# lordzuko/SpeakingStyle

Hardware: AMD Instinct MI355X
Metric: train mel-frames/sec (node) (higher is better)
Workload: dtype bf16; 1 GPU; model=FastSpeech2 (LJSpeech model.yaml), global_batch=200, seq_len=T~LJSpeech phonemes, M<=1000 mel frames, parallelism=dp1

## Files before the change

csrc/build.py:

```python
#!/usr/bin/env python
import argparse
import concurrent.futures as cf
import glob
import os
import subprocess
import sys
import sysconfig

HERE = os.path.dirname(os.path.abspath(__file__))
ROOT = os.path.dirname(HERE)
OUT_DIR = os.path.join(ROOT, "speakingstyle_amd", "_lib")
OBJ_DIR = os.path.join(ROOT, "build", "obj")
KLIB = os.path.join(OUT_DIR, "libssamd_kernels.so")
HLIB = os.path.join(OUT_DIR, "libssamd_host.so")
FLIB = os.path.join(OUT_DIR, "ssamd_fast" + sysconfig.get_config_var("EXT_SUFFIX"))
ARCH = os.environ.get("SSAMD_ARCH", "gfx950")
HIPCC = os.environ.get("HIPCC", "/opt/rocm/bin/hipcc")


def _run(cmd):
    r = subprocess.run(cmd, stdout=subprocess.PIPE, stderr=subprocess.STDOUT, text=True)
    if r.returncode != 0:
        raise RuntimeError("command failed: %s\n%s" % (" ".join(cmd), r.stdout))
    return r.stdout
# ... 26 lines not shown
    if clean or _stale(KLIB, objs):
        _run([HIPCC, "-shared", f"--offload-arch={ARCH}", "-Wl,-soname,libssamd_kernels.so", "-o", KLIB] + objs)

    build_fastcall(clean)

    hsrcs = sorted(glob.glob(os.path.join(HERE, "host_*.cpp")))
    if hsrcs and (clean or _stale(HLIB, hsrcs + headers)):
        _run(["g++", "-O3", "-std=c++17", "-fPIC", "-shared", "-pthread", "-o", HLIB] + hsrcs)
    if verbose:
        print("built", KLIB, FLIB, HLIB if hsrcs else "")
    return KLIB


def build_fastcall(clean=False):
    sys.path.insert(0, ROOT)
    sys.path.insert(0, HERE)
    import gen_fastcall

    src = gen_fastcall.generate(*gen_fastcall.signatures())
    gen_dir = os.path.join(ROOT, "build", "gen")
    os.makedirs(gen_dir, exist_ok=True)
    cpp = os.path.join(gen_dir, "ssamd_fast.cpp")
    old = open(cpp).read() if os.path.exists(cpp) else None
    if old != src:
        with open(cpp, "w") as f:
            f.write(src)
    if clean or _stale(FLIB, [cpp, KLIB]):
        inc = sysconfig.get_paths()["include"]
        _run(["g++", "-O2", "-std=c++17", "-fPIC", "-shared", "-I", inc, "-o", FLIB, cpp, "-L", OUT_DIR,
              "-l:libssamd_kernels.so", "-Wl,-rpath,$ORIGIN"])
    return FLIB


SANITIZERS = {"asan": ["-fsanitize=address,undefined", "-fno-sanitize-recover=all", "-fno-omit-frame-pointer"],
              "tsan": ["-fsanitize=thread"]}


def build_sanitized(verbose=False):
    out_dir = os.path.join(ROOT, "build", "sanitize")
    os.makedirs(out_dir, exist_ok=True)
    hsrcs = sorted(glob.glob(os.path.join(HERE, "host_*.cpp")))
    test = os.path.join(HERE, "selftest_host_collate.cpp")
    exes = {}
    for name, flags in SANITIZERS.items():
        exe = os.path.join(out_dir, f"selftest_host_{name}")
        if _stale(exe, hsrcs + [test]):
            _run(["g++", "-O1", "-g", "-std=c++17", "-pthread"] + flags + ["-o", exe, test] + hsrcs)
        exes[name] = exe
    if verbose:
        print("built", " ".join(exes.values()))
    return exes


def build_blockmap_selftest():
    out_dir = os.path.join(ROOT, "build", "sanitize")
    os.makedirs(out_dir, exist_ok=True)
    test = os.path.join(HERE, "selftest_attn_blockmap.cpp")
    exe = os.path.join(out_dir, "selftest_attn_blockmap")
    if _stale(exe, [test, os.path.join(HERE, "attn_blockmap.h")]):
        _run(["g++", "-O1", "-g", "-std=c++17", "-I", HERE] + SANITIZERS["asan"] + ["-o", exe, test])
    return exe


def build_gl_selftest():
    out_dir = os.path.join(ROOT, "build", "sanitize")
    os.makedirs(out_dir, exist_ok=True)
    test = os.path.join(HERE, "selftest_gl_frames.cpp")
    exe = os.path.join(out_dir, "selftest_gl_frames")
    if _stale(exe, [test, os.path.join(HERE, "gl_frames.h")]):
        _run(["g++", "-O1", "-g", "-std=c++17", "-I", HERE] + SANITIZERS["asan"] + ["-o", exe, test])
    return exe


def build_dtw_selftest():
    out_dir = os.path.join(ROOT, "build", "sanitize")
    os.makedirs(out_dir, exist_ok=True)
    test = os.path.join(HERE, "selftest_dtw_index.cpp")
    exe = os.path.join(out_dir, "selftest_dtw_index")
    if _stale(exe, [test, os.path.join(HERE, "dtw_index.h")]):
        _run(["g++", "-O1", "-g", "-std=c++17", "-I", HERE] + SANITIZERS["asan"] + ["-o", exe, test])
    return exe


if __name__ == "__main__":
    ap = argparse.ArgumentParser()
    ap.add_argument("--jobs", type=int, default=min(8, os.cpu_count() or 4))
    ap.add_argument("--debug", action="store_true")
    ap.add_argument("--clean", action="store_true")
    ap.add_argument("--sanitize", action="store_true",
                    help="also build the host runtime self-test under ASan+UBSan and TSan (build/sanitize/)")
    a = ap.parse_args()
    try:
        build(a.jobs, a.debug, a.clean, verbose=True)
        if a.sanitize:
            build_sanitized(verbose=True)
    except RuntimeError as e:
        print(e, file=sys.stderr)
        sys.exit(1)
```

csrc/k_gemm.hip:

```cpp
#include <mutex>
#include "common.h"
#include <type_traits>

namespace {

constexpr int BM = 128, BN = 128, BK = 64;
constexpr int NT = 256;
constexpr int CSTRIDE = 132;

struct ConvGeom {
  int B, L, Cin, ks, dil, pad;
  int M, N, K;
  const int2* rinfo;
  const int64_t* cu;
  int nseq;
  int prio;
  int ngrp;
  int ksplit;
};

__device__ __forceinline__ int2 tile_of(int T, int nM, int nN, int ngrp) {
  if (ngrp > 1) {
    const int per = nN / ngrp, gs = nM * per;
    const int grp = T / gs, r = T - grp * gs;
    return make_int2(r / per, grp * per + r % per);
  }
  return make_int2(T / nN, T % nN);
}

__device__ __forceinline__ int2 row_pos(const ConvGeom& g, int m) {
  if (g.rinfo) return g.rinfo[m];
  const int b = m / g.L;
  return make_int2(m - b * g.L, g.L);
}

enum { ACT_NONE = 0, ACT_RELU = 1, ACT_LRELU = 2, ACT_TANH = 3 };

struct EpiX {
  const bf16_t* acc;
  bf16_t* y2;
  float scale;
  int post_act;
  const float* bn_stats;
  float* bn_part;
  float bn_p;
  unsigned long long bn_seed;
  unsigned char* mask_out;
  const unsigned char* mask_in;
};

__device__ __forceinline__ int xcd_remap(int bid, int nwg) {
  const int q = nwg / 8, r = nwg % 8, xcd = bid % 8, k = bid / 8;
  return (xcd < r ? xcd * (q + 1) : r * (q + 1) + (xcd - r) * q) + k;
}

__device__ __forceinline__ int swz128(int row, int c) { return row * 128 + ((c ^ ((row >> 1) & 7)) << 4); }

__device__ __forceinline__ short8 load_a_chunk(const bf16_t* __restrict__ X, const ConvGeom& g, int m, int tt, int lim,
                                               int k, float invCin) {
  short8 v = {0, 0, 0, 0, 0, 0, 0, 0};
  if (m < g.M && k < g.K) {
    const int tap = (int)(((float)k + 0.5f) * invCin);
    const int cin = k - tap * g.Cin;
    const int sh = tap * g.dil - g.pad;
    const int ts = tt + sh;
    if (ts >= 0 && ts < lim) v = *reinterpret_cast<const short8*>(X + ((long)m + sh) * g.Cin + cin);
  }
  return v;
}

template <bool OUT_F32>
__device__ __forceinline__ void epi4x4_prefetch(const float4v (&acc)[4][4], int mb, int nb, int lane, const ConvGeom& g,
                                                const float* __restrict__ bias, const bf16_t* __restrict__ aux,
                                                const bf16_t* __restrict__ resid, const int64_t* __restrict__ lens,
                                                int act, int ldy, void* __restrict__ Yv) {
  float4 bvj[4];
  short4v xa[4][4], xr[4][4];
  bool vrow[4];
#pragma unroll
  for (int j = 0; j < 4; ++j) {
    const int n = nb + j * 16 + 4 * (lane >> 4);
    bvj[j] = (bias && n < g.N) ? *reinterpret_cast<const float4*>(bias + n) : make_float4(0.f, 0.f, 0.f, 0.f);
  }
#pragma unroll
// ... 192 lines not shown
      if (aux) {
        short8 x = *reinterpret_cast<const short8*>(aux + off);
#pragma unroll
        for (int q = 0; q < 8; ++q) v[q] = bf2f((bf16_t)x[q]) > 0.f ? v[q] : 0.f;
      }
      if (resid) {
        short8 x = *reinterpret_cast<const short8*>(resid + off);
#pragma unroll
        for (int q = 0; q < 8; ++q) v[q] += bf2f((bf16_t)x[q]);
      }
      if (!valid) {
#pragma unroll
        for (int q = 0; q < 8; ++q) v[q] = 0.f;
      }
      if constexpr (OUT_F32) {
        float4* Y = reinterpret_cast<float4*>(reinterpret_cast<float*>(Yv) + off);
        Y[0] = make_float4(v[0], v[1], v[2], v[3]);
        Y[1] = make_float4(v[4], v[5], v[6], v[7]);
      } else {
        short8 o;
#pragma unroll
        for (int q = 0; q < 8; ++q) o[q] = (short)f2bf(v[q]);
        *reinterpret_cast<short8*>(reinterpret_cast<bf16_t*>(Yv) + off) = o;
      }
    } else {
      for (int q = 0; q < 8; ++q) {
        if (nb + q >= g.N) break;
        float x = v[q];
        if (aux && !(bf2f(aux[off + q]) > 0.f)) x = 0.f;
        if (resid) x += bf2f(resid[off + q]);
        if (!valid) x = 0.f;
        if constexpr (OUT_F32) reinterpret_cast<float*>(Yv)[off + q] = x;
        else reinterpret_cast<bf16_t*>(Yv)[off + q] = f2bf(x);
      }
    }
  }
}

__device__ __attribute__((aligned(16))) bf16_t g_zero_chunk_mem[8];
__device__ __forceinline__ const void* zero_chunk_ptr() {
  const void* p = g_zero_chunk_mem;
  asm volatile("" : "+s"(p));
  return p;
}

__device__ __forceinline__ void glds16(const void* src, char* lds_wave_base) {
  __builtin_amdgcn_global_load_lds((const __attribute__((address_space(1))) void*)src,
                                   (__attribute__((address_space(3))) void*)lds_wave_base, 16, 0, 0);
}
__device__ __forceinline__ void buf_lds16(__amdgpu_buffer_rsrc_t r, int voff, int soff, char* lds_wave_base) {
  __builtin_amdgcn_raw_ptr_buffer_load_lds(r, (__attribute__((address_space(3))) void*)lds_wave_base, 16, voff, soff,
                                           0, 0);
}

template <bool OUT_F32>
__global__ void __launch_bounds__(NT, 2) conv_gemm_glds_kernel(const bf16_t* __restrict__ X, const bf16_t* __restrict__ W,
                                                               const float* __restrict__ bias,
                                                               const bf16_t* __restrict__ aux,
                                                               const bf16_t* __restrict__ resid,
                                                               const int64_t* __restrict__ lens, void* __restrict__ Yv,
                                                               ConvGeom g, int act, int ldy) {
  const void* const g_zero_chunk = zero_chunk_ptr();
  extern __shared__ __attribute__((aligned(16))) char smem[];
  const int nN = (g.N + BN - 1) / BN;
  const int nM = (g.M + BM - 1) / BM;
  const int wg = xcd_remap(blockIdx.x, nN * nM);
  const int tn = wg % nN, tm = wg / nN;
  const int m0 = tm * BM, n0 = tn * BN;
  const int tid = threadIdx.x, lane = tid & 63, wave = __builtin_amdgcn_readfirstlane(tid >> 6);
  const int wm = wave >> 1, wn = wave & 1;
  const float invCin = 1.f / (float)g.Cin;

  int a_lim[4], a_t[4], a_m[4], rowi[4], lchunk[4];
#pragma unroll
  for (int i = 0; i < 4; ++i) {
    const int row = (i * 4 + wave) * 8 + (lane >> 3);
    rowi[i] = row;
    lchunk[i] = (lane & 7) ^ ((row >> 1) & 7);
    a_m[i] = m0 + row;
    const int2 rp = row_pos(g, a_m[i] < g.M ? a_m[i] : 0);
    a_t[i] = rp.x;
    a_lim[i] = rp.y;
  }
  auto stage = [&](int kt, int buf) {
    char* As = smem + buf * (2 * BM * BK * 2);
    char* Bs = As + BM * BK * 2;
#pragma unroll
    for (int i = 0; i < 4; ++i) {
      const int k = kt * BK + lchunk[i] * 8;
      const void* src = g_zero_chunk;
      if (a_m[i] < g.M && k < g.K) {
        const int tap = (int)(((float)k + 0.5f) * invCin);
        const int cin = k - tap * g.Cin;
        const int sh = tap * g.dil - g.pad;
        const int ts = a_t[i] + sh;
        if (ts >= 0 && ts < a_lim[i]) src = X + ((long)a_m[i] + sh) * g.Cin + cin;
      }
      glds16(src, As + (i * 4 + wave) * 8 * 128);
      const int n = n0 + rowi[i];
      const void* srcb = (n < g.N && k < g.K) ? (const void*)(W + (long)n * g.K + k) : (const void*)g_zero_chunk;
      glds16(srcb, Bs + (i * 4 + wave) * 8 * 128);
    }
  };

  float4v acc[4][4];
#pragma unroll
  for (int i = 0; i < 4; ++i)
#pragma unroll
    for (int j = 0; j < 4; ++j) acc[i][j] = (float4v){0.f, 0.f, 0.f, 0.f};

  const int nk = (g.K + BK - 1) / BK;
  stage(0, 0);
  asm volatile("s_waitcnt vmcnt(0)" ::: "memory");
  __syncthreads();
  for (int kt = 0; kt < nk; ++kt) {
    const int buf = kt & 1;
    if (kt + 1 < nk) stage(kt + 1, buf ^ 1);
    const char* As = smem + buf * (2 * BM * BK * 2);
    const char* Bs = As + BM * BK * 2;
#pragma unroll
    for (int kk = 0; kk < 2; ++kk) {
      short8 fa[4], fb[4];
      const int c = kk * 4 + (lane >> 4);
#pragma unroll
      for (int i = 0; i < 4; ++i) {
        fa[i] = *reinterpret_cast<const short8*>(As + swz128(wm * 64 + i * 16 + (lane & 15), c));
        fb[i] = *reinterpret_cast<const short8*>(Bs + swz128(wn * 64 + i * 16 + (lane & 15), c));
      }
#pragma unroll
      for (int i = 0; i < 4; ++i)
#pragma unroll
        for (int j = 0; j < 4; ++j) acc[i][j] = __builtin_amdgcn_mfma_f32_16x16x32_bf16(fb[j], fa[i], acc[i][j], 0, 0, 0);
    }
    asm volatile("s_waitcnt vmcnt(0)" ::: "memory");
    __syncthreads();
  }
  epi4x4_prefetch<OUT_F32>(acc, m0 + wm * 64, n0 + wn * 64, lane, g, bias, aux, resid, lens, act, ldy, Yv);
}

constexpr int BM3 = 256, NT3 = 512, NSTAGE = 3;
constexpr int STAGE_BYTES = (BM3 + BN) * BK * 2;

template <bool OUT_F32, bool FASTK, bool PACKED, bool BUF = false>
__global__ void __launch_bounds__(NT3, 1) conv_gemm_ring_kernel(const bf16_t* __restrict__ X, const bf16_t* __restrict__ W,
                                                                const float* __restrict__ bias,
                                                                const bf16_t* __restrict__ aux,
                                                                const bf16_t* __restrict__ resid,
                                                                const int64_t* __restrict__ lens, void* __restrict__ Yv,
                                                                ConvGeom g, int act, int ldy, EpiX ex) {
  const void* const g_zero_chunk = zero_chunk_ptr();
  extern __shared__ __attribute__((aligned(16))) char smem[];
  const int nN = (g.N + BN - 1) / BN;
  const int nM = (g.M + BM3 - 1) / BM3;
  const int wg = xcd_remap(blockIdx.x, nN * nM);
  const int tn = wg % nN, tm = wg / nN;
  const int m0 = tm * BM3, n0 = tn * BN;
  const int tid = threadIdx.x, lane = tid & 63, wave = __builtin_amdgcn_readfirstlane(tid >> 6);
  const int wm = wave >> 1, wn = wave & 1;
  const float invCin = 1.f / (float)g.Cin;

  int a_lim[4], a_t[4], a_m[4], achunk[4];
  const bf16_t* arow_ptr[4];
  const bf16_t* brow_ptr[2];
  bool a_ok[4], b_ok[2];
#pragma unroll
  for (int i = 0; i < 4; ++i) {
    const int row = (i * 8 + wave) * 8 + (lane >> 3);
    achunk[i] = (lane & 7) ^ ((row >> 1) & 7);
    a_m[i] = m0 + row;
    a_ok[i] = a_m[i] < g.M;
    const int mm = a_ok[i] ? a_m[i] : 0;
    if constexpr (PACKED) {
      const int2 rp = g.rinfo[mm];
      a_t[i] = rp.x;
      a_lim[i] = rp.y;
    } else {
      const int bb = mm / g.L;
      a_t[i] = mm - bb * g.L;
      a_lim[i] = g.L;
    }
    arow_ptr[i] = X + (long)mm * g.Cin + achunk[i] * 8;
  }
#pragma unroll
  for (int i = 0; i < 2; ++i) {
    const int row = (i * 8 + wave) * 8 + (lane >> 3);
    const int bch = (lane & 7) ^ ((row >> 1) & 7);
    const int n = n0 + row;
    b_ok[i] = n < g.N;
    brow_ptr[i] = W + (long)(b_ok[i] ? n : 0) * g.K + bch * 8;
  }
  constexpr int kOOB = (int)0x80000000;
  const __amdgpu_buffer_rsrc_t rA = __builtin_amdgcn_make_buffer_rsrc(
      (void*)(X - (long)g.pad * g.Cin), 0, BUF ? (g.M + g.pad) * g.Cin * 2 : 0, 0x00020000);
  const __amdgpu_buffer_rsrc_t rB = __builtin_amdgcn_make_buffer_rsrc((void*)W, 0, BUF ? g.N * g.K * 2 : 0,
                                                                      0x00020000);
  int avo[4], bvo[2];
  if constexpr (BUF) {
#pragma unroll
    for (int i = 0; i < 4; ++i) avo[i] = a_ok[i] ? ((a_m[i] + g.pad) * g.Cin + achunk[i] * 8) * 2 : kOOB;
#pragma unroll
    for (int i = 0; i < 2; ++i) {
      const int row = (i * 8 + wave) * 8 + (lane >> 3);
      const int bch = (lane & 7) ^ ((row >> 1) & 7);
      bvo[i] = b_ok[i] ? ((n0 + row) * g.K + bch * 8) * 2 : kOOB;
    }
  }
  auto stage = [&](int kt, int buf) {
    char* As = smem + buf * STAGE_BYTES;
    char* Bs = As + BM3 * BK * 2;
    const int k0 = kt * BK;
    if constexpr (BUF) {
      const int tap = k0 / g.Cin;
      const int cin0 = k0 - tap * g.Cin;
      const int shift = tap * g.dil - g.pad;
      const int aoff = (shift * g.Cin + cin0) * 2;
#pragma unroll
      for (int i = 0; i < 4; ++i) {
        const int ts = a_t[i] + shift;
        const bool ok = (unsigned)ts < (unsigned)a_lim[i];
        buf_lds16(rA, ok ? avo[i] + aoff : kOOB, 0, As + (i * 8 + wave) * 8 * 128);
      }
#pragma unroll
      for (int i = 0; i < 2; ++i) buf_lds16(rB, bvo[i], k0 * 2, Bs + (i * 8 + wave) * 8 * 128);
    } else if constexpr (FASTK) {
      const int tap = k0 / g.Cin;
      const int cin0 = k0 - tap * g.Cin;
      const int shift = tap * g.dil - g.pad;
      const long off = (long)shift * g.Cin + cin0;
#pragma unroll
      for (int i = 0; i < 4; ++i) {
        const int ts = a_t[i] + shift;
        const bool ok = a_ok[i] && (unsigned)ts < (unsigned)a_lim[i];
        glds16(ok ? (const void*)(arow_ptr[i] + off) : (const void*)g_zero_chunk, As + (i * 8 + wave) * 8 * 128);
      }
#pragma unroll
      for (int i = 0; i < 2; ++i)
        glds16(b_ok[i] ? (const void*)(brow_ptr[i] + k0) : (const void*)g_zero_chunk, Bs + (i * 8 + wave) * 8 * 128);
    } else {
#pragma unroll
      for (int i = 0; i < 4; ++i) {
        const int k = k0 + achunk[i] * 8;
        const void* src = g_zero_chunk;
        if (a_ok[i] && k < g.K) {
          const int tap = (int)(((float)k + 0.5f) * invCin);
          const int cin = k - tap * g.Cin;
          const int sh = tap * g.dil - g.pad;
          const int ts = a_t[i] + sh;
          if (ts >= 0 && ts < a_lim[i]) src = arow_ptr[i] - achunk[i] * 8 + (long)sh * g.Cin + cin;
        }
        glds16(src, As + (i * 8 + wave) * 8 * 128);
      }
#pragma unroll
      for (int i = 0; i < 2; ++i) {
        const int row = (i * 8 + wave) * 8 + (lane >> 3);
        const int k = k0 + ((lane & 7) ^ ((row >> 1) & 7)) * 8;
        glds16((b_ok[i] && k < g.K) ? (const void*)(brow_ptr[i] + k0) : (const void*)g_zero_chunk,
               Bs + (i * 8 + wave) * 8 * 128);
      }
    }
  };

  float4v acc[4][4];
#pragma unroll
  for (int i = 0; i < 4; ++i)
#pragma unroll
    for (int j = 0; j < 4; ++j) acc[i][j] = (float4v){0.f, 0.f, 0.f, 0.f};

  const int nk = (g.K + BK - 1) / BK;
  stage(0, 0);
  if (nk > 1) {
    stage(1, 1);
    asm volatile("s_waitcnt vmcnt(6)" ::: "memory");
  } else {
    asm volatile("s_waitcnt vmcnt(0)" ::: "memory");
  }
  __builtin_amdgcn_s_barrier();
  int buf = 0;
  for (int kt = 0; kt < nk; ++kt) {
    if (kt + 2 < nk) stage(kt + 2, (buf + 2) % NSTAGE);
    const char* As = smem + buf * STAGE_BYTES;
    const char* Bs = As + BM3 * BK * 2;
#pragma unroll
    for (int kk = 0; kk < 2; ++kk) {
      short8 fa[4], fb[4];
      const int c = kk * 4 + (lane >> 4);
#pragma unroll
      for (int i = 0; i < 4; ++i) {
        fa[i] = *reinterpret_cast<const short8*>(As + swz128(wm * 64 + i * 16 + (lane & 15), c));
        fb[i] = *reinterpret_cast<const short8*>(Bs + swz128(wn * 64 + i * 16 + (lane & 15), c));
      }
#pragma unroll
      for (int i = 0; i < 4; ++i)
#pragma unroll
        for (int j = 0; j < 4; ++j) acc[i][j] = __builtin_amdgcn_mfma_f32_16x16x32_bf16(fb[j], fa[i], acc[i][j], 0, 0, 0);
    }
    if (kt + 2 < nk) asm volatile("s_waitcnt vmcnt(6) lgkmcnt(0)" ::: "memory");
    else asm volatile("s_waitcnt vmcnt(0) lgkmcnt(0)" ::: "memory");
    __builtin_amdgcn_s_barrier();
    buf = (buf + 1) % NSTAGE;
  }
  float4 bvj[4];
  short4v xa[4][4], xr[4][4], xc[4][4];
  bool vrow[4];
#pragma unroll
  for (int j = 0; j < 4; ++j) {
    const int n = n0 + wn * 64 + j * 16 + 4 * (lane >> 4);
    bvj[j] = (bias && n < g.N) ? *reinterpret_cast<const float4*>(bias + n) : make_float4(0.f, 0.f, 0.f, 0.f);
  }
#pragma unroll
  for (int i = 0; i < 4; ++i) {
    const int m = m0 + wm * 64 + i * 16 + (lane & 15);
    const int mm = m < g.M ? m : 0;
    const int bb = mm / g.L, tt = mm - bb * g.L;
    vrow[i] = lens == nullptr || tt < (int)lens[bb];
#pragma unroll
    for (int j = 0; j < 4; ++j) {
      const int n = n0 + wn * 64 + j * 16 + 4 * (lane >> 4);
      const bool in = m < g.M && n < g.N;
      const long off = (long)m * ldy + n;
      if (in && aux) xa[i][j] = *reinterpret_cast<const short4v*>(aux + off);
// ... 108 lines not shown
    *reinterpret_cast<short4v*>(reinterpret_cast<bf16_t*>(Yv) + off) = o;
  }
}

constexpr int STG64_BYTES = 2 * BG * 64 * 2;
constexpr int B64_LDS = 256 * 528;

__device__ __forceinline__ void pp_barrier() {
  asm volatile("" ::: "memory");
  __builtin_amdgcn_sched_barrier(0);
  __builtin_amdgcn_s_barrier();
  __builtin_amdgcn_sched_barrier(0);
  asm volatile("" ::: "memory");
}

constexpr int EPI_GEN = 0, EPI_BNH = 1, EPI_MASK = 2;

__device__ __forceinline__ int ct_woff(int ml, int nl) { return ml * 528 + ((nl * 2) ^ (((ml >> 3) & 1) << 3)); }
__device__ __forceinline__ short8 ct_read(const char* Ct, int r, int c16) {
  const short8 v = *reinterpret_cast<const short8*>(Ct + r * 528 + c16 * 16);
  return ((r >> 3) & 1) ? __builtin_shufflevector(v, v, 4, 5, 6, 7, 0, 1, 2, 3) : v;
}
template <bool OUT_F32, bool FASTK, bool PACKED, bool BUF, int EPIM, bool STG>
__device__ __forceinline__ void big64_tile(const bf16_t* __restrict__ X, const bf16_t* __restrict__ W,
                                           const float* __restrict__ bias, const bf16_t* __restrict__ aux,
                                           const bf16_t* __restrict__ resid, const int64_t* __restrict__ lens,
                                           void* __restrict__ Yv, ConvGeom g, int act, int ldy, EpiX ex, int vb) {
  const void* const g_zero_chunk = zero_chunk_ptr();
  extern __shared__ __attribute__((aligned(16))) char smem[];
  const int nN = (g.N + BG - 1) / BG;
  const int nM = (g.M + BG - 1) / BG;
  const int2 tmn = tile_of(xcd_remap(vb, nN * nM), nM, nN, g.ngrp);
  const int tm = tmn.x, tn = tmn.y;
  const int m0 = tm * BG, n0 = tn * BG;
  const int tid = threadIdx.x, lane = tid & 63, wave = __builtin_amdgcn_readfirstlane(tid >> 6);
  const int wm = wave >> 2, wn = wave & 3;
  const float invCin = 1.f / (float)g.Cin;
  if (g.prio && wave >= 4) __builtin_amdgcn_s_setprio(1);

  int a_lim[4], a_t[4], a_m[4], achunk[4];
  const bf16_t* arow_ptr[4];
  const bf16_t* brow_ptr[4];
  bool a_ok[4], b_ok[4];
  int2 rp[4];
#pragma unroll
  for (int i = 0; i < 4; ++i) {
    const int row = (i * 8 + wave) * 8 + (lane >> 3);
    achunk[i] = (lane & 7) ^ ((row >> 1) & 7);
    a_m[i] = m0 + row;
    a_ok[i] = a_m[i] < g.M;
    if constexpr (PACKED) rp[i] = g.rinfo[a_ok[i] ? a_m[i] : 0];
  }
#pragma unroll
  for (int i = 0; i < 4; ++i) {
    const int mm = a_ok[i] ? a_m[i] : 0;
    if constexpr (PACKED) {
      a_t[i] = rp[i].x;
      a_lim[i] = rp[i].y;
    } else {
      const int bb = mm / g.L;
      a_t[i] = mm - bb * g.L;
      a_lim[i] = g.L;
    }
    arow_ptr[i] = X + (long)mm * g.Cin + achunk[i] * 8;
    const int row = (i * 8 + wave) * 8 + (lane >> 3);
    const int n = n0 + row;
    b_ok[i] = n < g.N;
    brow_ptr[i] = W + (long)(b_ok[i] ? n : 0) * g.K + achunk[i] * 8;
  }
  constexpr int kOOB = (int)0x80000000;
  const __amdgpu_buffer_rsrc_t rA = __builtin_amdgcn_make_buffer_rsrc(
      (void*)(X - (long)g.pad * g.Cin), 0, BUF ? (g.M + g.pad) * g.Cin * 2 : 0, 0x00020000);
  const __amdgpu_buffer_rsrc_t rB = __builtin_amdgcn_make_buffer_rsrc((void*)W, 0, BUF ? g.N * g.K * 2 : 0,
                                                                      0x00020000);
  int avo[4], bvo[4];
  if constexpr (BUF) {
#pragma unroll
    for (int i = 0; i < 4; ++i) {
      avo[i] = a_ok[i] ? ((a_m[i] + g.pad) * g.Cin + achunk[i] * 8) * 2 : kOOB;
      const int row = (i * 8 + wave) * 8 + (lane >> 3);
      bvo[i] = b_ok[i] ? ((n0 + row) * g.K + achunk[i] * 8) * 2 : kOOB;
    }
  }
  auto stage = [&](int kt, int buf) {
    char* As = smem + buf * STG64_BYTES;
    char* Bs = As + BG * 64 * 2;
    const int k0 = kt * 64;
    if constexpr (BUF) {
      const int tap = k0 / g.Cin;
      const int cin0 = k0 - tap * g.Cin;
      const int shift = tap * g.dil - g.pad;
      const int aoff = (shift * g.Cin + cin0) * 2;
#pragma unroll
      for (int i = 0; i < 4; ++i) {
        const int ts = a_t[i] + shift;
        const bool ok = (unsigned)ts < (unsigned)a_lim[i];
        buf_lds16(rA, ok ? avo[i] + aoff : kOOB, 0, As + (i * 8 + wave) * 1024);
      }
#pragma unroll
      for (int i = 0; i < 4; ++i) buf_lds16(rB, bvo[i], k0 * 2, Bs + (i * 8 + wave) * 1024);
    } else if constexpr (FASTK) {
      const int tap = k0 / g.Cin;
      const int cin0 = k0 - tap * g.Cin;
      const int shift = tap * g.dil - g.pad;
      const long off = (long)shift * g.Cin + cin0;
#pragma unroll
      for (int i = 0; i < 4; ++i) {
        const int ts = a_t[i] + shift;
        const bool ok = a_ok[i] && (unsigned)ts < (unsigned)a_lim[i];
        glds16(ok ? (const void*)(arow_ptr[i] + off) : (const void*)g_zero_chunk, As + (i * 8 + wave) * 1024);
      }
#pragma unroll
      for (int i = 0; i < 4; ++i)
        glds16(b_ok[i] ? (const void*)(brow_ptr[i] + k0) : (const void*)g_zero_chunk, Bs + (i * 8 + wave) * 1024);
    } else {
#pragma unroll
      for (int i = 0; i < 4; ++i) {
        const int k = k0 + achunk[i] * 8;
        const void* src = g_zero_chunk;
        if (a_ok[i] && k < g.K) {
          const int tap = (int)(((float)k + 0.5f) * invCin);
          const int cin = k - tap * g.Cin;
          const int sh = tap * g.dil - g.pad;
          const int ts = a_t[i] + sh;
          if (ts >= 0 && ts < a_lim[i]) src = arow_ptr[i] - achunk[i] * 8 + (long)sh * g.Cin + cin;
        }
        glds16(src, As + (i * 8 + wave) * 1024);
      }
#pragma unroll
      for (int i = 0; i < 4; ++i) {
        const int k = k0 + achunk[i] * 8;
        glds16((b_ok[i] && k < g.K) ? (const void*)(brow_ptr[i] + k0) : (const void*)g_zero_chunk,
               Bs + (i * 8 + wave) * 1024);
      }
    }
  };

  float4v acc[8][4];
#pragma unroll
  for (int i = 0; i < 8; ++i)
#pragma unroll
    for (int j = 0; j < 4; ++j) acc[i][j] = (float4v){0.f, 0.f, 0.f, 0.f};

  unsigned char mpre[16];
  if constexpr (EPIM == EPI_MASK) {
    const int c = tid & 31, r0 = tid >> 5;
    const int n = n0 + c * 8;
#pragma unroll
    for (int it = 0; it < 16; ++it) {
      const int m = m0 + r0 + 16 * it;
      mpre[it] = (n < g.N && m < g.M) ? ex.mask_in[(long)m * (g.N >> 3) + (n >> 3)] : (unsigned char)0;
    }
  }
  constexpr int BNH_PRE = STG ? 8 : 16;
  short8 hpre[16];
  auto load_h = [&](int it0, int it1) {
    const int c = tid & 31, r0 = tid >> 5;
    const int n = n0 + c * 8;
#pragma unroll
    for (int it = it0; it < it1; ++it) {
      const int m = m0 + r0 + 16 * it;
      hpre[it] = (short8){0, 0, 0, 0, 0, 0, 0, 0};
      if (n < g.N && m < g.M) hpre[it] = *reinterpret_cast<const short8*>(ex.acc + (long)m * ldy + n);
    }
  };
  if constexpr (EPIM == EPI_BNH) {
    load_h(0, BNH_PRE);
  }
  const int nk_all = (g.K + 63) / 64;
  int kt0 = 0, nk = nk_all;
  if (gridDim.y > 1) {
    const int per = (nk_all + gridDim.y - 1) / gridDim.y;
    kt0 = blockIdx.y * per;
    nk = min(nk_all, kt0 + per);
    Yv = reinterpret_cast<float*>(Yv) + (long)blockIdx.y * g.M * ldy;
  }
  if (g.ksplit > 0 && gridDim.y == 1) {
    const int kc = g.Cin / 64;
    if (n0 < g.ksplit) nk = 2 * kc;
    else kt0 = kc;
  }
  if constexpr (STG) {
    int bblk[4], bvo2[4];
    bblk[0] = 8 * (wave >> 2) + (wave & 3);
    bblk[1] = bblk[0] + 16;
    bblk[2] = bblk[0] + 4;
    bblk[3] = bblk[1] + 4;
#pragma unroll
    for (int u = 0; u < 4; ++u) {
      const int row = bblk[u] * 8 + (lane >> 3);
      const int ch = (lane & 7) ^ ((row >> 1) & 7);
      bvo2[u] = (n0 + row < g.N) ? ((n0 + row) * g.K + ch * 8) * 2 : kOOB;
    }
    auto stage_a = [&](int kt, int q, int buf) {
      char* As = smem + buf * STG64_BYTES;
      const int k0 = kt * 64;
      const int tap = k0 / g.Cin;
      const int cin0 = k0 - tap * g.Cin;
      const int shift = tap * g.dil - g.pad;
      const int aoff = (shift * g.Cin + cin0) * 2;
#pragma unroll
      for (int jj = 0; jj < 2; ++jj) {
        const int i = q + 2 * jj;
        const int ts = a_t[i] + shift;
        const bool ok = (unsigned)ts < (unsigned)a_lim[i];
        buf_lds16(rA, ok ? avo[i] + aoff : kOOB, 0, As + (i * 8 + wave) * 1024);
      }
    };
    auto stage_b = [&](int kt, int q, int buf) {
      char* Bs = smem + buf * STG64_BYTES + BG * 64 * 2;
#pragma unroll
      for (int jj = 0; jj < 2; ++jj) buf_lds16(rB, bvo2[q * 2 + jj], kt * 128, Bs + bblk[q * 2 + jj] * 1024);
    };
    short8 fa[2][4], fb0[2][2], fb1[2][2];
    auto read_a = [&](const char* As, int qa) {
#pragma unroll
      for (int kk = 0; kk < 2; ++kk) {
        const int c = kk * 4 + (lane >> 4);
#pragma unroll
        for (int i = 0; i < 4; ++i)
          fa[kk][i] = *reinterpret_cast<const short8*>(As + swz128(wm * 128 + qa * 64 + i * 16 + (lane & 15), c));
      }
    };
    auto read_b = [&](const char* Bs, int qb, short8 (&fb)[2][2]) {
#pragma unroll
      for (int kk = 0; kk < 2; ++kk) {
        const int c = kk * 4 + (lane >> 4);
#pragma unroll
        for (int j = 0; j < 2; ++j)
          fb[kk][j] = *reinterpret_cast<const short8*>(Bs + swz128(wn * 64 + qb * 32 + j * 16 + (lane & 15), c));
      }
    };
    auto mma = [&](int qa, int qb, const short8 (&fb)[2][2]) {
      asm volatile("s_waitcnt lgkmcnt(0)" ::: "memory");
      __builtin_amdgcn_sched_barrier(0);
      __builtin_amdgcn_s_setprio(1);
#pragma unroll
      for (int kk = 0; kk < 2; ++kk)
#pragma unroll
        for (int i = 0; i < 4; ++i)
#pragma unroll
          for (int j = 0; j < 2; ++j)
            acc[qa * 4 + i][qb * 2 + j] =
                __builtin_amdgcn_mfma_f32_16x16x32_bf16(fb[kk][j], fa[kk][i], acc[qa * 4 + i][qb * 2 + j], 0, 0, 0);
      __builtin_amdgcn_s_setprio(0);
    };
    const int nkt = nk - kt0;
    if (nkt > 0) { stage_a(kt0, 0, 0); stage_b(kt0, 1, 0); stage_a(kt0, 1, 0); stage_b(kt0, 0, 0); }
    if (nkt > 1) {
      stage_a(kt0 + 1, 0, 1); stage_b(kt0 + 1, 1, 1); stage_a(kt0 + 1, 1, 1); stage_b(kt0 + 1, 0, 1);
      asm volatile("s_waitcnt vmcnt(8)" ::: "memory");
    } else {
      asm volatile("s_waitcnt vmcnt(0)" ::: "memory");
    }
    pp_barrier();
    if (wm == 1) pp_barrier();
    for (int t = 0; t < nkt; ++t) {
      const int buf = t & 1, kt = kt0 + t;
      const char* As = smem + buf * STG64_BYTES;
      const char* Bs = As + BG * 64 * 2;
      const bool s1 = t >= 1 && t + 1 < nkt;
      const bool s2 = t + 2 < nkt;
      if (s1) stage_a(kt + 1, 1, buf ^ 1);
      read_a(As, 0);
      read_b(Bs, 0, fb0);
      pp_barrier();
      mma(0, 0, fb0);
      pp_barrier();
      if (s1) stage_b(kt + 1, 0, buf ^ 1);
      read_b(Bs, 1, fb1);
      pp_barrier();
      mma(0, 1, fb1);
      pp_barrier();
      if (s2) stage_a(kt + 2, 0, buf);
      read_a(As, 1);
      pp_barrier();
      mma(1, 1, fb1);
      pp_barrier();
      if (s2) stage_b(kt + 2, 1, buf);
      if (t + 1 < nkt) {
        if (s2) asm volatile("s_waitcnt vmcnt(4)" ::: "memory");
        else asm volatile("s_waitcnt vmcnt(0)" ::: "memory");
      }
      pp_barrier();
      mma(1, 0, fb0);
      pp_barrier();
    }
    if (wm == 0) pp_barrier();
    asm volatile("s_waitcnt vmcnt(0)" ::: "memory");
    pp_barrier();
  } else {
  if (kt0 < nk) stage(kt0, 0);
  asm volatile("s_waitcnt vmcnt(0)" ::: "memory");
  __builtin_amdgcn_s_barrier();
  for (int kt = kt0; kt < nk; ++kt) {
    const int buf = (kt - kt0) & 1;
    if (kt + 1 < nk) stage(kt + 1, buf ^ 1);
    const char* As = smem + buf * STG64_BYTES;
    const char* Bs = As + BG * 64 * 2;
#pragma unroll
    for (int kk = 0; kk < 2; ++kk) {
      const int c = kk * 4 + (lane >> 4);
      short8 fa[8], fb[4];
#pragma unroll
      for (int j = 0; j < 4; ++j) fb[j] = *reinterpret_cast<const short8*>(Bs + swz128(wn * 64 + j * 16 + (lane & 15), c));
#pragma unroll
      for (int i = 0; i < 8; ++i) fa[i] = *reinterpret_cast<const short8*>(As + swz128(wm * 128 + i * 16 + (lane & 15), c));
#pragma unroll
      for (int i = 0; i < 8; ++i)
#pragma unroll
        for (int j = 0; j < 4; ++j) acc[i][j] = __builtin_amdgcn_mfma_f32_16x16x32_bf16(fb[j], fa[i], acc[i][j], 0, 0, 0);
    }
    asm volatile("s_waitcnt vmcnt(0) lgkmcnt(0)" ::: "memory");
    __builtin_amdgcn_s_barrier();
  }
  }
  if constexpr (!OUT_F32) {
    if (act >= 0 && (g.N & 7) == 0 && (ldy & 7) == 0) {
      char* Ct = smem;
      auto stage_tile = [&](auto actc, auto biasc) {
        constexpr int A = decltype(actc)::value;
        constexpr bool HB = decltype(biasc)::value;
        float4 bv[4];
        if constexpr (HB) {
#pragma unroll
          for (int j = 0; j < 4; ++j) {
            const int n = n0 + wn * 64 + j * 16 + 4 * (lane >> 4);
            bv[j] = n < g.N ? *reinterpret_cast<const float4*>(bias + n) : make_float4(0.f, 0.f, 0.f, 0.f);
          }
        }
#pragma unroll
        for (int i = 0; i < 8; ++i) {
          const int ml = wm * 128 + i * 16 + (lane & 15);
#pragma unroll
          for (int j = 0; j < 4; ++j) {
            const int nl = wn * 64 + j * 16 + 4 * (lane >> 4);
            float v[4] = {acc[i][j][0], acc[i][j][1], acc[i][j][2], acc[i][j][3]};
            if constexpr (HB) {
              v[0] += bv[j].x; v[1] += bv[j].y; v[2] += bv[j].z; v[3] += bv[j].w;
            }
            if constexpr (A == ACT_RELU) {
#pragma unroll
              for (int q = 0; q < 4; ++q) v[q] = fmaxf(v[q], 0.f);
            } else if constexpr (A == ACT_LRELU) {
#pragma unroll
              for (int q = 0; q < 4; ++q) v[q] = v[q] > 0.f ? v[q] : 0.1f * v[q];
            } else if constexpr (A == ACT_TANH) {
#pragma unroll
              for (int q = 0; q < 4; ++q) v[q] = tanhf(v[q]);
            }
            short4v o;
#pragma unroll
            for (int q = 0; q < 4; ++q) o[q] = (short)f2bf(v[q]);
            *reinterpret_cast<short4v*>(Ct + ct_woff(ml, nl)) = o;
          }
        }
      };
      auto stage_act = [&](auto biasc) {
        if (act == ACT_RELU) stage_tile(std::integral_constant<int, ACT_RELU>{}, biasc);
        else if (act == ACT_LRELU) stage_tile(std::integral_constant<int, ACT_LRELU>{}, biasc);
        else if (act == ACT_TANH) stage_tile(std::integral_constant<int, ACT_TANH>{}, biasc);
        else stage_tile(std::integral_constant<int, ACT_NONE>{}, biasc);
      };
      if constexpr (EPIM == EPI_BNH) stage_tile(std::integral_constant<int, ACT_NONE>{}, std::false_type{});
      else if (bias) stage_act(std::true_type{});
      else stage_act(std::false_type{});
      if constexpr (EPIM == EPI_BNH) {
        if constexpr (BNH_PRE < 16) load_h(BNH_PRE, 16);
      }
// ... 1817 lines not shown
```

Before: 4.535 million mel-frames/s.

## Walk conv-GEMM K dimension chunk-major across taps to reuse activation rows

Adds a K-walk helper that orders the implicit-GEMM conv reduction chunk-major (all taps for one 64-channel chunk before moving on) unless ksplit needs tap-major order. It also adds a fast path in the generic stage that uses tap and chunk counters instead of float division per element, and advances slab counters incrementally in the pipelined kernel. Consecutive K steps then touch the same channel chunk of shifted activation rows, which is meant to improve cache reuse and cut the per-step index arithmetic. The accumulation order changes, so bf16/fp32 results may differ slightly. A host self-test for the walk is included.

```diff
diff --git a/csrc/build.py b/csrc/build.py
--- a/csrc/build.py
+++ b/csrc/build.py
@@ -132,6 +132,16 @@
     return exe
 
 
+def build_kwalk_selftest():
+    out_dir = os.path.join(ROOT, "build", "sanitize")
+    os.makedirs(out_dir, exist_ok=True)
+    test = os.path.join(HERE, "selftest_gemm_kwalk.cpp")
+    exe = os.path.join(out_dir, "selftest_gemm_kwalk")
+    if _stale(exe, [test, os.path.join(HERE, "gemm_kwalk.h")]):
+        _run(["g++", "-O1", "-g", "-std=c++17", "-I", HERE] + SANITIZERS["asan"] + ["-o", exe, test])
+    return exe
+
+
 if __name__ == "__main__":
     ap = argparse.ArgumentParser()
     ap.add_argument("--jobs", type=int, default=min(8, os.cpu_count() or 4))
diff --git a/csrc/gemm_kwalk.h b/csrc/gemm_kwalk.h
--- /dev/null
+++ b/csrc/gemm_kwalk.h
@@ -0,0 +1,54 @@
+#pragma once
+
+#if defined(__HIPCC__) || defined(__CUDACC__)
+#define KWALK_HD __host__ __device__
+#else
+#define KWALK_HD
+#endif
+
+#define KWALK_SLAB 64
+
+struct KSlab {
+  int tap;
+  int chunk;
+};
+
+KWALK_HD inline int kwalk_num_slabs(int Cin, int ks) { return ks * (Cin / KWALK_SLAB); }
+
+KWALK_HD inline KSlab kwalk_slab(int kt, int Cin, int ks, bool tap_major) {
+  KSlab s;
+  if (tap_major) {
+    const int kc = Cin / KWALK_SLAB;
+    s.tap = kt / kc;
+    s.chunk = kt - s.tap * kc;
+  } else {
+    s.chunk = kt / ks;
+    s.tap = kt - s.chunk * ks;
+  }
+  return s;
+}
+
+KWALK_HD inline KSlab kwalk_next(KSlab s, int Cin, int ks, bool tap_major) {
+  if (tap_major) {
+    if (++s.chunk == Cin / KWALK_SLAB) { s.chunk = 0; ++s.tap; }
+  } else {
+    if (++s.tap == ks) { s.tap = 0; ++s.chunk; }
+  }
+  return s;
+}
+
+KWALK_HD inline int kwalk_b_offset(KSlab s, int Cin) { return s.tap * Cin + s.chunk * KWALK_SLAB; }
+KWALK_HD inline int kwalk_a_shift(KSlab s, int dil, int pad) { return s.tap * dil - pad; }
+KWALK_HD inline int kwalk_a_channel(KSlab s) { return s.chunk * KWALK_SLAB; }
+
+KWALK_HD inline void kwalk_slice(int nk, int S, int y, int* kt0, int* kt1) {
+  const int per = (nk + S - 1) / S;
+  *kt0 = y * per < nk ? y * per : nk;
+  *kt1 = *kt0 + per < nk ? *kt0 + per : nk;
+}
+
+KWALK_HD inline void kwalk_ksplit_range(int Cin, bool low, int* kt0, int* kt1) {
+  const int kc = Cin / KWALK_SLAB;
+  *kt0 = low ? 0 : kc;
+  *kt1 = low ? 2 * kc : 3 * kc;
+}
diff --git a/csrc/k_gemm.hip b/csrc/k_gemm.hip
--- a/csrc/k_gemm.hip
+++ b/csrc/k_gemm.hip
@@ -1,5 +1,6 @@
 #include <mutex>
 #include "common.h"
+#include "gemm_kwalk.h"
 #include <type_traits>
 
 namespace {
@@ -358,9 +359,27 @@
     a_t[i] = rp.x;
     a_lim[i] = rp.y;
   }
+  const bool fastk = g.Cin % BK == 0;
   auto stage = [&](int kt, int buf) {
     char* As = smem + buf * (2 * BM * BK * 2);
     char* Bs = As + BM * BK * 2;
+    if (fastk) {
+      const KSlab sl = kwalk_slab(kt, g.Cin, g.ks, g.ksplit > 0);
+      const int shift = kwalk_a_shift(sl, g.dil, g.pad);
+      const long off = (long)shift * g.Cin + kwalk_a_channel(sl);
+      const int boff = kwalk_b_offset(sl, g.Cin);
+#pragma unroll
+      for (int i = 0; i < 4; ++i) {
+        const int ts = a_t[i] + shift;
+        const bool ok = a_m[i] < g.M && (unsigned)ts < (unsigned)a_lim[i];
+        glds16(ok ? (const void*)(X + (long)a_m[i] * g.Cin + off + lchunk[i] * 8) : g_zero_chunk,
+               As + (i * 4 + wave) * 8 * 128);
+        const int n = n0 + rowi[i];
+        glds16(n < g.N ? (const void*)(W + (long)n * g.K + boff + lchunk[i] * 8) : g_zero_chunk,
+               Bs + (i * 4 + wave) * 8 * 128);
+      }
+      return;
+    }
 #pragma unroll
     for (int i = 0; i < 4; ++i) {
       const int k = kt * BK + lchunk[i] * 8;
@@ -486,32 +505,32 @@
     char* Bs = As + BM3 * BK * 2;
     const int k0 = kt * BK;
     if constexpr (BUF) {
-      const int tap = k0 / g.Cin;
-      const int cin0 = k0 - tap * g.Cin;
-      const int shift = tap * g.dil - g.pad;
-      const int aoff = (shift * g.Cin + cin0) * 2;
+      const KSlab sl = kwalk_slab(kt, g.Cin, g.ks, g.ksplit > 0);
+      const int shift = kwalk_a_shift(sl, g.dil, g.pad);
+      const int aoff = (shift * g.Cin + kwalk_a_channel(sl)) * 2;
 #pragma unroll
       for (int i = 0; i < 4; ++i) {
         const int ts = a_t[i] + shift;
         const bool ok = (unsigned)ts < (unsigned)a_lim[i];
         buf_lds16(rA, ok ? avo[i] + aoff : kOOB, 0, As + (i * 8 + wave) * 8 * 128);
       }
-#pragma unroll
-      for (int i = 0; i < 2; ++i) buf_lds16(rB, bvo[i], k0 * 2, Bs + (i * 8 + wave) * 8 * 128);
+      const int boff = kwalk_b_offset(sl, g.Cin) * 2;
+#pragma unroll
+      for (int i = 0; i < 2; ++i) buf_lds16(rB, bvo[i], boff, Bs + (i * 8 + wave) * 8 * 128);
     } else if constexpr (FASTK) {
-      const int tap = k0 / g.Cin;
-      const int cin0 = k0 - tap * g.Cin;
-      const int shift = tap * g.dil - g.pad;
-      const long off = (long)shift * g.Cin + cin0;
+      const KSlab sl = kwalk_slab(kt, g.Cin, g.ks, g.ksplit > 0);
+      const int shift = kwalk_a_shift(sl, g.dil, g.pad);
+      const long off = (long)shift * g.Cin + kwalk_a_channel(sl);
 #pragma unroll
       for (int i = 0; i < 4; ++i) {
         const int ts = a_t[i] + shift;
         const bool ok = a_ok[i] && (unsigned)ts < (unsigned)a_lim[i];
         glds16(ok ? (const void*)(arow_ptr[i] + off) : (const void*)g_zero_chunk, As + (i * 8 + wave) * 8 * 128);
       }
+      const int boff = kwalk_b_offset(sl, g.Cin);
 #pragma unroll
       for (int i = 0; i < 2; ++i)
-        glds16(b_ok[i] ? (const void*)(brow_ptr[i] + k0) : (const void*)g_zero_chunk, Bs + (i * 8 + wave) * 8 * 128);
+        glds16(b_ok[i] ? (const void*)(brow_ptr[i] + boff) : (const void*)g_zero_chunk, Bs + (i * 8 + wave) * 8 * 128);
     } else {
 #pragma unroll
       for (int i = 0; i < 4; ++i) {
@@ -786,37 +805,38 @@
       bvo[i] = b_ok[i] ? ((n0 + row) * g.K + achunk[i] * 8) * 2 : kOOB;
     }
   }
+  const bool tapmaj = g.ksplit > 0;
   auto stage = [&](int kt, int buf) {
     char* As = smem + buf * STG64_BYTES;
     char* Bs = As + BG * 64 * 2;
     const int k0 = kt * 64;
     if constexpr (BUF) {
-      const int tap = k0 / g.Cin;
-      const int cin0 = k0 - tap * g.Cin;
-      const int shift = tap * g.dil - g.pad;
-      const int aoff = (shift * g.Cin + cin0) * 2;
+      const KSlab sl = kwalk_slab(kt, g.Cin, g.ks, tapmaj);
+      const int shift = kwalk_a_shift(sl, g.dil, g.pad);
+      const int aoff = (shift * g.Cin + kwalk_a_channel(sl)) * 2;
 #pragma unroll
       for (int i = 0; i < 4; ++i) {
         const int ts = a_t[i] + shift;
         const bool ok = (unsigned)ts < (unsigned)a_lim[i];
         buf_lds16(rA, ok ? avo[i] + aoff : kOOB, 0, As + (i * 8 + wave) * 1024);
       }
-#pragma unroll
-      for (int i = 0; i < 4; ++i) buf_lds16(rB, bvo[i], k0 * 2, Bs + (i * 8 + wave) * 1024);
+      const int boff = kwalk_b_offset(sl, g.Cin) * 2;
+#pragma unroll
+      for (int i = 0; i < 4; ++i) buf_lds16(rB, bvo[i], boff, Bs + (i * 8 + wave) * 1024);
     } else if constexpr (FASTK) {
-      const int tap = k0 / g.Cin;
-      const int cin0 = k0 - tap * g.Cin;
-      const int shift = tap * g.dil - g.pad;
-      const long off = (long)shift * g.Cin + cin0;
+      const KSlab sl = kwalk_slab(kt, g.Cin, g.ks, tapmaj);
+      const int shift = kwalk_a_shift(sl, g.dil, g.pad);
+      const long off = (long)shift * g.Cin + kwalk_a_channel(sl);
 #pragma unroll
       for (int i = 0; i < 4; ++i) {
         const int ts = a_t[i] + shift;
         const bool ok = a_ok[i] && (unsigned)ts < (unsigned)a_lim[i];
         glds16(ok ? (const void*)(arow_ptr[i] + off) : (const void*)g_zero_chunk, As + (i * 8 + wave) * 1024);
       }
+      const int boff = kwalk_b_offset(sl, g.Cin);
 #pragma unroll
       for (int i = 0; i < 4; ++i)
-        glds16(b_ok[i] ? (const void*)(brow_ptr[i] + k0) : (const void*)g_zero_chunk, Bs + (i * 8 + wave) * 1024);
+        glds16(b_ok[i] ? (const void*)(brow_ptr[i] + boff) : (const void*)g_zero_chunk, Bs + (i * 8 + wave) * 1024);
     } else {
 #pragma unroll
       for (int i = 0; i < 4; ++i) {
@@ -874,16 +894,10 @@
   const int nk_all = (g.K + 63) / 64;
   int kt0 = 0, nk = nk_all;
   if (gridDim.y > 1) {
-    const int per = (nk_all + gridDim.y - 1) / gridDim.y;
-    kt0 = blockIdx.y * per;
-    nk = min(nk_all, kt0 + per);
+    kwalk_slice(nk_all, gridDim.y, blockIdx.y, &kt0, &nk);
     Yv = reinterpret_cast<float*>(Yv) + (long)blockIdx.y * g.M * ldy;
   }
-  if (g.ksplit > 0 && gridDim.y == 1) {
-    const int kc = g.Cin / 64;
-    if (n0 < g.ksplit) nk = 2 * kc;
-    else kt0 = kc;
-  }
+  if (g.ksplit > 0 && gridDim.y == 1) kwalk_ksplit_range(g.Cin, n0 < g.ksplit, &kt0, &nk);
   if constexpr (STG) {
     int bblk[4], bvo2[4];
     bblk[0] = 8 * (wave >> 2) + (wave & 3);
@@ -896,13 +910,10 @@
       const int ch = (lane & 7) ^ ((row >> 1) & 7);
       bvo2[u] = (n0 + row < g.N) ? ((n0 + row) * g.K + ch * 8) * 2 : kOOB;
     }
-    auto stage_a = [&](int kt, int q, int buf) {
+    auto stage_a = [&](KSlab sl, int q, int buf) {
       char* As = smem + buf * STG64_BYTES;
-      const int k0 = kt * 64;
-      const int tap = k0 / g.Cin;
-      const int cin0 = k0 - tap * g.Cin;
-      const int shift = tap * g.dil - g.pad;
-      const int aoff = (shift * g.Cin + cin0) * 2;
+      const int shift = kwalk_a_shift(sl, g.dil, g.pad);
+      const int aoff = (shift * g.Cin + kwalk_a_channel(sl)) * 2;
 #pragma unroll
       for (int jj = 0; jj < 2; ++jj) {
         const int i = q + 2 * jj;
@@ -911,10 +922,11 @@
         buf_lds16(rA, ok ? avo[i] + aoff : kOOB, 0, As + (i * 8 + wave) * 1024);
       }
     };
-    auto stage_b = [&](int kt, int q, int buf) {
+    auto stage_b = [&](KSlab sl, int q, int buf) {
       char* Bs = smem + buf * STG64_BYTES + BG * 64 * 2;
-#pragma unroll
-      for (int jj = 0; jj < 2; ++jj) buf_lds16(rB, bvo2[q * 2 + jj], kt * 128, Bs + bblk[q * 2 + jj] * 1024);
+      const int boff = kwalk_b_offset(sl, g.Cin) * 2;
+#pragma unroll
+      for (int jj = 0; jj < 2; ++jj) buf_lds16(rB, bvo2[q * 2 + jj], boff, Bs + bblk[q * 2 + jj] * 1024);
     };
     short8 fa[2][4], fb0[2][2], fb1[2][2];
     auto read_a = [&](const char* As, int qa) {
@@ -950,9 +962,12 @@
       __builtin_amdgcn_s_setprio(0);
     };
     const int nkt = nk - kt0;
-    if (nkt > 0) { stage_a(kt0, 0, 0); stage_b(kt0, 1, 0); stage_a(kt0, 1, 0); stage_b(kt0, 0, 0); }
+    const KSlab sl0 = kwalk_slab(kt0, g.Cin, g.ks, tapmaj);
+    KSlab sl1 = kwalk_next(sl0, g.Cin, g.ks, tapmaj);
+    KSlab sl2 = kwalk_next(sl1, g.Cin, g.ks, tapmaj);
+    if (nkt > 0) { stage_a(sl0, 0, 0); stage_b(sl0, 1, 0); stage_a(sl0, 1, 0); stage_b(sl0, 0, 0); }
     if (nkt > 1) {
-      stage_a(kt0 + 1, 0, 1); stage_b(kt0 + 1, 1, 1); stage_a(kt0 + 1, 1, 1); stage_b(kt0 + 1, 0, 1);
+      stage_a(sl1, 0, 1); stage_b(sl1, 1, 1); stage_a(sl1, 1, 1); stage_b(sl1, 0, 1);
       asm volatile("s_waitcnt vmcnt(8)" ::: "memory");
     } else {
       asm volatile("s_waitcnt vmcnt(0)" ::: "memory");
@@ -960,28 +975,28 @@
     pp_barrier();
     if (wm == 1) pp_barrier();
     for (int t = 0; t < nkt; ++t) {
-      const int buf = t & 1, kt = kt0 + t;
+      const int buf = t & 1;
       const char* As = smem + buf * STG64_BYTES;
       const char* Bs = As + BG * 64 * 2;
       const bool s1 = t >= 1 && t + 1 < nkt;
       const bool s2 = t + 2 < nkt;
-      if (s1) stage_a(kt + 1, 1, buf ^ 1);
+      if (s1) stage_a(sl1, 1, buf ^ 1);
       read_a(As, 0);
       read_b(Bs, 0, fb0);
       pp_barrier();
       mma(0, 0, fb0);
       pp_barrier();
-      if (s1) stage_b(kt + 1, 0, buf ^ 1);
+      if (s1) stage_b(sl1, 0, buf ^ 1);
       read_b(Bs, 1, fb1);
       pp_barrier();
       mma(0, 1, fb1);
       pp_barrier();
-      if (s2) stage_a(kt + 2, 0, buf);
+      if (s2) stage_a(sl2, 0, buf);
       read_a(As, 1);
       pp_barrier();
       mma(1, 1, fb1);
       pp_barrier();
-      if (s2) stage_b(kt + 2, 1, buf);
+      if (s2) stage_b(sl2, 1, buf);
       if (t + 1 < nkt) {
         if (s2) asm volatile("s_waitcnt vmcnt(4)" ::: "memory");
         else asm volatile("s_waitcnt vmcnt(0)" ::: "memory");
@@ -989,6 +1004,8 @@
       pp_barrier();
       mma(1, 0, fb0);
       pp_barrier();
+      sl1 = sl2;
+      sl2 = kwalk_next(sl2, g.Cin, g.ks, tapmaj);
     }
     if (wm == 0) pp_barrier();
     asm volatile("s_waitcnt vmcnt(0)" ::: "memory");
diff --git a/csrc/selftest_gemm_kwalk.cpp b/csrc/selftest_gemm_kwalk.cpp
--- /dev/null
+++ b/csrc/selftest_gemm_kwalk.cpp
@@ -0,0 +1,107 @@
+#include <cstdio>
+#include <vector>
+
+#include "gemm_kwalk.h"
+
+static int fails = 0;
+#define CHECK(c, ...)                         \
+  do {                                        \
+    if (!(c)) {                               \
+      if (++fails <= 20) {                    \
+        std::printf("FAIL %s: ", #c);         \
+        std::printf(__VA_ARGS__);             \
+        std::printf("\n");                    \
+      }                                       \
+    }                                         \
+  } while (0)
+
+static void check_walk(int Cin, int ks, bool tap_major) {
+  const int kc = Cin / KWALK_SLAB, nk = kwalk_num_slabs(Cin, ks), K = ks * Cin;
+  CHECK(nk == K / 64, "Cin %d ks %d: %d slabs", Cin, ks, nk);
+  std::vector<int> seen((size_t)ks * kc, 0);
+  std::vector<unsigned char> wrow((size_t)K, 0);
+  KSlab run = kwalk_slab(0, Cin, ks, tap_major), prev = run;
+  for (int kt = 0; kt < nk; ++kt) {
+    const KSlab s = kwalk_slab(kt, Cin, ks, tap_major);
+    CHECK(s.tap >= 0 && s.tap < ks && s.chunk >= 0 && s.chunk < kc, "Cin %d ks %d tm %d: slab %d -> (%d, %d)", Cin, ks,
+          tap_major, kt, s.tap, s.chunk);
+    if (s.tap < 0 || s.tap >= ks || s.chunk < 0 || s.chunk >= kc) return;
+    CHECK(run.tap == s.tap && run.chunk == s.chunk, "Cin %d ks %d tm %d: counters (%d, %d) at slab %d, walk (%d, %d)",
+          Cin, ks, tap_major, run.tap, run.chunk, kt, s.tap, s.chunk);
+    CHECK(!seen[(size_t)s.tap * kc + s.chunk], "Cin %d ks %d tm %d: (%d, %d) twice", Cin, ks, tap_major, s.tap, s.chunk);
+    seen[(size_t)s.tap * kc + s.chunk] = 1;
+    if (!tap_major) {
+      CHECK(s.tap == kt % ks && s.chunk == kt / ks, "Cin %d ks %d: slab %d", Cin, ks, kt);
+      if (kt > 0 && s.tap != 0)
+        CHECK(s.chunk == prev.chunk && s.tap == prev.tap + 1, "Cin %d ks %d: slab %d leaves its chunk early", Cin, ks, kt);
+      if (kt > 0 && s.tap == 0)
+        CHECK(prev.tap == ks - 1 && s.chunk == prev.chunk + 1, "Cin %d ks %d: slab %d starts a chunk early", Cin, ks, kt);
+    } else {
+      CHECK(s.tap == kt * 64 / Cin && s.chunk * 64 == kt * 64 - s.tap * Cin, "Cin %d ks %d: tap-major slab %d", Cin, ks, kt);
+    }
+    if (ks == 1) CHECK(s.tap == 0 && s.chunk == kt, "Cin %d: ks 1 is not the identity at slab %d", Cin, kt);
+    const int bo = kwalk_b_offset(s, Cin);
+    CHECK(bo >= 0 && bo + KWALK_SLAB <= K && bo % KWALK_SLAB == 0, "Cin %d ks %d: B offset %d of %d", Cin, ks, bo, K);
+    if (bo < 0 || bo + KWALK_SLAB > K) return;
+    for (int e = 0; e < KWALK_SLAB; ++e) {
+      CHECK(!wrow[(size_t)bo + e], "Cin %d ks %d: weight element %d staged twice", Cin, ks, bo + e);
+      wrow[(size_t)bo + e] = 1;
+    }
+    CHECK(bo == s.tap * Cin + kwalk_a_channel(s), "Cin %d ks %d: A channel and B offset disagree", Cin, ks);
+    for (int dil : {1, 3, 5}) {
+      const int pad = dil * (ks - 1) / 2;
+      const int sh = kwalk_a_shift(s, dil, pad);
+      CHECK(sh == s.tap * dil - pad && sh >= -pad && sh <= pad, "Cin %d ks %d dil %d: shift %d", Cin, ks, dil, sh);
+    }
+    prev = s;
+    run = kwalk_next(run, Cin, ks, tap_major);
+  }
+  for (int e = 0; e < K; ++e) CHECK(wrow[(size_t)e], "Cin %d ks %d: weight element %d never staged", Cin, ks, e);
+
+  for (int S = 1; S <= 8; ++S) {
+    int at = 0;
+    for (int y = 0; y < S; ++y) {
+      int k0, k1;
+      kwalk_slice(nk, S, y, &k0, &k1);
+      CHECK(k0 == at && k1 >= k0 && k1 <= nk, "nk %d S %d: slice %d = [%d, %d), expected start %d", nk, S, y, k0, k1, at);
+      const int per = (nk + S - 1) / S, p0 = y * per, p1 = nk < p0 + per ? nk : p0 + per;
+      CHECK((p0 >= p1 && k0 == k1) || (p0 == k0 && p1 == k1), "nk %d S %d: slice %d differs from the formula", nk, S, y);
+      at = k1;
+    }
+    CHECK(at == nk, "nk %d S %d: slices end at %d", nk, S, at);
+  }
+}
+
+static void check_ksplit(int Cin) {
+  const int kc = Cin / KWALK_SLAB;
+  for (int low = 0; low < 2; ++low) {
+    int k0, k1;
+    kwalk_ksplit_range(Cin, low != 0, &k0, &k1);
+    int p0 = 0, p1 = 3 * kc;
+    if (low) p1 = 2 * kc;
+    else p0 = kc;
+    CHECK(k0 == p0 && k1 == p1, "Cin %d low %d: [%d, %d) vs [%d, %d)", Cin, low, k0, k1, p0, p1);
+    for (int kt = 0; kt < 3 * kc; ++kt) {
+      const KSlab s = kwalk_slab(kt, Cin, 3, true);
+      const bool in = kt >= k0 && kt < k1, want = low ? s.tap <= 1 : s.tap >= 1;
+      CHECK(in == want, "Cin %d low %d: slab %d (tap %d) %s", Cin, low, kt, s.tap, in ? "kept" : "skipped");
+    }
+  }
+}
+
+int main() {
+  int walks = 0;
+  for (int ks : {1, 3, 5, 7, 9, 11})
+    for (int kc : {1, 2, 4, 8, 16})
+      for (int tm = 0; tm < 2; ++tm) {
+        check_walk(kc * 64, ks, tm != 0);
+        ++walks;
+      }
+  for (int kc : {1, 2, 4, 8, 16}) check_ksplit(kc * 64);
+  if (fails) {
+    std::printf("selftest_gemm_kwalk: %d failures\n", fails);
+    return 1;
+  }
+  std::printf("selftest_gemm_kwalk ok (%d walks)\n", walks);
+  return 0;
+}
```

Result: no change. 4.574 million mel-frames/s, median of 6 (+0.8%).
